# DiltheyLab/MetaMaps

Measured on AMD Instinct MI355X. Metric: Gbp long reads mapped+classified per sec (whole node), miniSeq+H DB, higher is better.
Workload: dtype u32

## Files before the change

### include/metamaps_hip.h

```cpp
#ifndef METAMAPS_HIP_H
#define METAMAPS_HIP_H

#include <stddef.h>
#include <stdint.h>

#ifdef __cplusplus
extern "C" {
#endif

#define MM_ABI_VERSION 6

typedef enum {
  MM_OK = 0,
  MM_ERR_ARG = -1,
  MM_ERR_DEVICE = -2,
  MM_ERR_NOMEM = -3,
  MM_ERR_STATE = -4,
  MM_ERR_LIMIT = -5,
  MM_ERR_NUMERIC = -6,
  MM_ERR_COMM = -7,
  MM_ERR_DATA = -8
} mm_status;

typedef struct mm_ctx mm_ctx;
// ... 130 lines not shown
  int64_t sum_sketch, sum_hits, n_candidates, sum_l2_stream_entries, sum_l2_evals;
  int64_t n_ambiguous_sketch_reads;
  int64_t sum_hits_kept;
  int64_t n_l2_rebuilds;
  int64_t n_l2_wide_redo;
  double ms_minimizer, ms_sketch, ms_probe_gather, ms_sort_hits, ms_l1_scan, ms_l2, ms_compact, ms_total, ms_hit_filter;
  int64_t n_reads_giant;
} mm_map_stats;

int mm_map_batch(mm_ctx* ctx, const mm_index* idx, const mm_seqset* reads, const mm_map_params* p, mm_mapping** out);
int mm_map_batch_phased(mm_ctx* ctx, const mm_index* idx, const mm_seqset* reads, const mm_map_params* p, void (*at_stage)(void* user, int stage), void* user,
                        mm_mapping** out);
int mm_map_batch_reusing(mm_ctx* ctx, const mm_index* idx, const mm_seqset* reads, const mm_map_params* p, const mm_mapping* sketch_of, mm_mapping** out);
int mm_sketch_batch(mm_ctx* ctx, const mm_seqset* reads, const mm_map_params* p, mm_mapping** out);
void mm_mapping_destroy(mm_mapping* m);
int mm_mapping_get_stats(const mm_mapping* m, mm_map_stats* out);
int mm_mapping_release_intermediates(mm_mapping* m);
int mm_mapping_fetch(mm_mapping* m, int64_t* offsets, mm_map_record* records, int64_t cap);
int mm_mapping_add_qualities(mm_ctx* ctx, mm_mapping* m, const mm_seqset* reads, int k);
int mm_mapping_keep_best(mm_ctx* ctx, mm_mapping* m, int k);
int mm_mapping_concat(mm_ctx* ctx, mm_mapping* const* parts, const int32_t* contig_base, int n_parts, mm_mapping** out);
int mm_mapping_from_parts(mm_ctx* ctx, int64_t n_reads, const int32_t* read_len, const mm_map_params* p, int n_parts,
                          const int64_t* const* offsets, const mm_map_record* const* records, const int32_t* contig_base, mm_mapping** out);

int mm_mapping_gather(mm_ctx* ctx, int owner, int64_t n_reads, const int32_t* read_len, const mm_map_params* p, mm_mapping* const* parts, const int32_t* chunk_id,
                      int n_parts, int n_chunks, const int32_t* chunk_rank, const int32_t* contig_base, mm_mapping** out);

int mm_debug_sketch(mm_mapping* m, int64_t* offsets, uint32_t* hash, int32_t* strand, int64_t cap);
int mm_debug_hits(mm_mapping* m, int64_t* offsets, int32_t* contig, int32_t* wpos, int64_t cap);
int mm_debug_candidates(mm_mapping* m, int64_t* offsets, int32_t* triples , int64_t cap);
int mm_debug_l2(mm_mapping* m, int64_t* per_cand , int64_t cap);
int mm_debug_min_hits(mm_mapping* m, int32_t* min_hits );
int mm_debug_probed_lists(mm_mapping* m, const mm_index* idx, int64_t* hist, int32_t n_bins);

int mm_em_create(mm_ctx* ctx, int64_t n_reads, const int64_t* read_off, const int32_t* taxon, const double* mapq,
                 const double* inv_nloc, int32_t n_taxa, mm_em** out);
int mm_em_create_from_mapping(mm_ctx* ctx, const mm_mapping* m, const int32_t* contig_taxon, const int32_t* contig_len, int32_t n_contigs,
                              int32_t n_taxa, mm_em** out);
int mm_em_taxon_counts(mm_em* em, int64_t* counts);
int mm_em_sizes(const mm_em* em, int64_t* n_reads, int64_t* n_entries, int32_t* n_taxa);
void mm_em_destroy(mm_em* em);
int mm_em_iterate(mm_em* em, const double* f, double* f_partial, double* ll_partial);
int mm_em_iterate_allreduce(mm_em* em, const double* f, double* f_next, double* ll);
int mm_em_run(mm_em* em, const double* f0, int max_iter, double* f_out, double* ll_trace, int ll_cap, int* n_iter);
int mm_em_continue(mm_em* em, int max_iter, double* f_out, double* ll_trace, int ll_cap, int* n_iter, int* stopped);
int mm_em_posteriors(mm_em* em, const double* f, double* post , int64_t* best );
int mm_em_bootstrap(mm_em* em, const double* f_start, int32_t rep0, int32_t n_rep, uint64_t seed, const uint8_t* weights,
                    int max_iter, double* f_out, double* ll_out, int32_t* n_iter, int32_t* stopped);
int mm_em_lca(mm_em* em, const double* f, int32_t n_nodes, const int32_t* parent, const int32_t* taxon_node, double threshold,
              int32_t* node_out, double* mass_out, int64_t* direct_out);

int mm_gene_overlap(mm_ctx* ctx, int32_t n_contigs, const int64_t* contig_gene_off, const int32_t* gene_start, const int32_t* gene_stop,
                    const int32_t* gene_group, int32_t n_groups,
                    const int64_t* group_feat_off , const int32_t* group_feat, int32_t n_feats,
                    int64_t n_maps, const int32_t* map_contig, const int32_t* map_start, const int32_t* map_stop, const double* map_ident,
                    int64_t* group_reads , double* group_median ,
                    int64_t* feat_reads , int64_t* maps_on_annotated );

#define MM_COMM_ID_BYTES 128
int mm_comm_unique_id(char id[MM_COMM_ID_BYTES]);
int mm_comm_init(mm_ctx* ctx, const char id[MM_COMM_ID_BYTES], int rank, int nranks);
int mm_comm_info(mm_ctx* ctx, int* n_ranks, int* rank);
int mm_comm_share(mm_ctx* ctx, mm_ctx* owner);
int mm_comm_allreduce_f64(mm_ctx* ctx, double* host_inout, int64_t n);
void mm_comm_destroy(mm_ctx* ctx);

// ... 5 lines not shown
```

### metamaps_amd/capi.py

```python
from __future__ import annotations

import ctypes as C
import os
import re

import numpy as np

_HERE = os.path.dirname(os.path.abspath(__file__))
LIB_PATH = os.path.join(_HERE, "csrc", "libmetamaps_hip.so")
HEADER_PATH = os.path.join(os.path.dirname(_HERE), "include", "metamaps_hip.h")

COMM_ID_BYTES = 128
MM_ERR_ARG = -1
MM_ERR_LIMIT = -5
MM_ERR_DATA = -8


class MMError(RuntimeError):
    def __init__(self, status: int, msg: str):
        super().__init__(f"libmetamaps_hip status {status}: {msg}")
        self.status = status


SEED_STAGE_CB = C.CFUNCTYPE(None, C.c_void_p, C.c_int)
# ... 114 lines not shown
            "mm_index_load": (C.c_int, [vp, C.c_char_p, P(vp)]),
            "mm_index_destroy": (None, [vp]),
            "mm_index_get_info": (C.c_int, [vp, P(IndexInfo)]),
            "mm_index_freq_hist": (C.c_int, [vp, vp, vp, i64, P(i64)]),
            "mm_freq_threshold_from_hist": (C.c_int, [vp, vp, i64, i64, C.c_int]),
            "mm_index_set_freq_threshold": (C.c_int, [vp, C.c_int]),
            "mm_index_entries": (C.c_int, [vp, vp, vp, vp, vp, i64]),
            "mm_index_dup_neighbours": (C.c_int, [vp, vp, vp, i64]),
            "mm_recommended_window": (C.c_int, [f64, C.c_int, f32, C.c_int, u64]),
            "mm_estimate_pvalue": (f64, [C.c_int, C.c_int, f32, C.c_int, u64]),
            "mm_min_hits_relaxed": (C.c_int, [C.c_int, C.c_int, f32]),
            "mm_identity": (None, [C.c_int, C.c_int, C.c_int, P(f32), P(f32)]),
            "mm_map_batch": (C.c_int, [vp, vp, vp, P(MapParams), P(vp)]),
            "mm_map_batch_phased": (C.c_int, [vp, vp, vp, P(MapParams), SEED_STAGE_CB, vp, P(vp)]),
            "mm_map_batch_reusing": (C.c_int, [vp, vp, vp, P(MapParams), vp, P(vp)]),
            "mm_sketch_batch": (C.c_int, [vp, vp, P(MapParams), P(vp)]),
            "mm_mapping_destroy": (None, [vp]),
            "mm_mapping_get_stats": (C.c_int, [vp, P(MapStats)]),
            "mm_comm_info": (C.c_int, [vp, C.POINTER(C.c_int), C.POINTER(C.c_int)]),
            "mm_mapping_gather": (C.c_int, [vp, C.c_int, i64, vp, vp, vp, vp, C.c_int, C.c_int, vp, vp, vp]),
            "mm_mapping_release_intermediates": (C.c_int, [vp]),
            "mm_mapping_fetch": (C.c_int, [vp, vp, vp, i64]),
            "mm_mapping_add_qualities": (C.c_int, [vp, vp, vp, C.c_int]),
            "mm_mapping_concat": (C.c_int, [vp, P(vp), vp, C.c_int, P(vp)]),
            "mm_mapping_keep_best": (C.c_int, [vp, vp, C.c_int]),
            "mm_mapping_from_parts": (C.c_int, [vp, i64, vp, P(MapParams), C.c_int, P(vp), P(vp), vp, P(vp)]),
            "mm_index_plan_chunks": (C.c_int, [vp, vp, u64, vp, i32, P(i32)]),
            "mm_debug_sketch": (C.c_int, [vp, vp, vp, vp, i64]),
            "mm_debug_hits": (C.c_int, [vp, vp, vp, vp, i64]),
            "mm_debug_candidates": (C.c_int, [vp, vp, vp, i64]),
            "mm_debug_l2": (C.c_int, [vp, vp, i64]),
            "mm_debug_min_hits": (C.c_int, [vp, vp]),
            "mm_debug_probed_lists": (C.c_int, [vp, vp, vp, i32]),
            "mm_em_create": (C.c_int, [vp, i64, vp, vp, vp, vp, i32, P(vp)]),
            "mm_em_create_from_mapping": (C.c_int, [vp, vp, vp, vp, i32, i32, P(vp)]),
            "mm_em_taxon_counts": (C.c_int, [vp, vp]),
            "mm_em_sizes": (C.c_int, [vp, P(i64), P(i64), P(i32)]),
            "mm_em_destroy": (None, [vp]),
            "mm_em_iterate": (C.c_int, [vp, vp, vp, P(f64)]),
            "mm_em_iterate_allreduce": (C.c_int, [vp, vp, vp, P(f64)]),
            "mm_em_posteriors": (C.c_int, [vp, vp, vp, vp]),
            "mm_em_run": (C.c_int, [vp, vp, C.c_int, vp, vp, C.c_int, P(C.c_int)]),
            "mm_em_continue": (C.c_int, [vp, C.c_int, vp, vp, C.c_int, P(C.c_int), P(C.c_int)]),
            "mm_em_bootstrap": (C.c_int, [vp, vp, i32, i32, u64, vp, C.c_int, vp, vp, vp, vp]),
            "mm_em_lca": (C.c_int, [vp, vp, i32, vp, vp, f64, vp, vp, vp]),
            "mm_gene_overlap": (C.c_int, [vp, i32, vp, vp, vp, vp, i32, vp, vp, i32, i64, vp, vp, vp, vp, vp, vp, vp, P(i64)]),
            "mm_comm_unique_id": (C.c_int, [C.c_char_p]),
            "mm_comm_init": (C.c_int, [vp, C.c_char_p, C.c_int, C.c_int]),
            "mm_comm_allreduce_f64": (C.c_int, [vp, vp, i64]),
            "mm_comm_share": (C.c_int, [vp, vp]),
            "mm_comm_destroy": (None, [vp]),
        }
        for name, (res, args) in sig.items():
            fn = getattr(L, name)
            fn.restype = res
            fn.argtypes = args
        _lib = L
    return _lib


def _ptr(a):
    return None if a is None else a.ctypes.data_as(C.c_void_p)


class Context:
    def __init__(self, device: int = 0):
# ... 463 lines not shown
        return off, h, s

    def debug_hits(self):
        off = np.zeros(self.n_reads + 1, dtype=np.int64)
        self.ctx.check(lib().mm_debug_hits(self.h, _ptr(off), None, None, 0))
        c = np.zeros(int(off[-1]), dtype=np.int32)
        w = np.zeros(int(off[-1]), dtype=np.int32)
        self.ctx.check(lib().mm_debug_hits(self.h, _ptr(off), _ptr(c), _ptr(w), len(c)))
        return off, c, w

    def debug_candidates(self):
        off = np.zeros(self.n_reads + 1, dtype=np.int64)
        self.ctx.check(lib().mm_debug_candidates(self.h, _ptr(off), None, 0))
        t = np.zeros((int(off[-1]), 3), dtype=np.int32)
        self.ctx.check(lib().mm_debug_candidates(self.h, _ptr(off), _ptr(t), len(t)))
        return off, t

    def debug_l2(self, n_cand: int):
        a = np.zeros((n_cand, 6), dtype=np.int64)
        if n_cand:
            self.ctx.check(lib().mm_debug_l2(self.h, _ptr(a), n_cand))
        return a

    def debug_min_hits(self):
        a = np.zeros(self.n_reads, dtype=np.int32)
        self.ctx.check(lib().mm_debug_min_hits(self.h, _ptr(a)))
        return a

    def debug_probed_lists(self, idx: "Index", n_bins: int = 66) -> np.ndarray:
        a = np.zeros(n_bins, dtype=np.int64)
        self.ctx.check(lib().mm_debug_probed_lists(self.h, idx.h, _ptr(a), n_bins))
        return a

    def close(self):
        if self.h:
            lib().mm_mapping_destroy(self.h)
            self.h = None


class EM:
    def __init__(self, ctx: Context, h, n_taxa: int, n_reads: int, n_entries: int, n_mapped: int | None = None):
        self.ctx, self.h, self.n_taxa, self.n_reads, self.n_entries = ctx, h, n_taxa, n_reads, n_entries
        self.n_mapped = n_mapped

    def iterate(self, f: np.ndarray):
        f = np.ascontiguousarray(f, dtype=np.float64)
        part = np.zeros(self.n_taxa, dtype=np.float64)
        ll = C.c_double()
        self.ctx.check(lib().mm_em_iterate(self.h, _ptr(f), _ptr(part), C.byref(ll)))
        return part, ll.value

    def iterate_allreduce(self, f: np.ndarray):
        f = np.ascontiguousarray(f, dtype=np.float64)
        nxt = np.zeros(self.n_taxa, dtype=np.float64)
        ll = C.c_double()
        self.ctx.check(lib().mm_em_iterate_allreduce(self.h, _ptr(f), _ptr(nxt), C.byref(ll)))
        return nxt, ll.value

    def run(self, f0: np.ndarray, max_iter: int = 1000):
        f0 = np.ascontiguousarray(f0, dtype=np.float64)
        f = np.zeros(self.n_taxa, dtype=np.float64)
        ll = np.zeros(1024, dtype=np.float64)
        n = C.c_int()
        self.ctx.check(lib().mm_em_run(self.h, _ptr(f0), max_iter, _ptr(f), _ptr(ll), len(ll), C.byref(n)))
        return f, ll[:min(n.value, len(ll))]

# ... 53 lines not shown
```

### metamaps_amd/csrc/mm_api.hip

```cpp
#include "mm_env.hpp"
#include "mm_map.hpp"
#include "mm_em.hpp"
#include "mm_stats.hpp"
#include "mm_synth.hpp"
#include "mm_hpc.hpp"
#include "mm_lca.hpp"
#include "mm_gene.hpp"
#include <chrono>
#include <new>
#include <rccl/rccl.h>
#include <rocprim/rocprim.hpp>

namespace mm {
void seqset_upload(mm_seqset* s);
void seqset_upload_nt16(mm_seqset* s);
int64_t bgzf_inflate(mm_ctx* ctx, const uint8_t* comp, int64_t comp_bytes, const int64_t* comp_off, const int32_t* comp_len, int32_t n,
                     uint8_t* out, int64_t out_cap, const int64_t* out_off, int32_t* status);
void bgzf_deflate(mm_ctx* ctx, const uint8_t* in, int64_t in_bytes, uint8_t* out, int64_t out_cap, int64_t* out_bytes, int32_t* n_blocks);
int64_t bgzf_deflate_bound(int64_t in_bytes);
mm_gzip* gzip_open(mm_ctx* ctx, int64_t chunk, int64_t segment);
void gzip_close(mm_gzip* g);
int gzip_feed(mm_gzip* g, const uint8_t* comp, int64_t n, bool last, int64_t* avail);
int64_t gzip_read(mm_gzip* g, uint8_t* out, int64_t cap);
void gzip_stats(const mm_gzip* g, int64_t* counts, double* seconds);
// ... 792 lines not shown
    if (!triples) return;
    MM_REQUIRE(cap >= m->n_cand, MM_ERR_ARG, "output capacity too small");
    m->cand.download(triples, (size_t)(3 * m->n_cand), m->ctx->stream);
    MM_HIP(mm::stream_sync(m->ctx->stream));
  });
}
int mm_debug_l2(mm_mapping* m, int64_t* per_cand, int64_t cap) {
  if (m && m->released) return MM_ERR_STATE;
  if (!m || !per_cand) return MM_ERR_ARG;
  return guarded(m->ctx, [&] {
    MM_REQUIRE(cap >= m->n_cand, MM_ERR_ARG, "output capacity too small");
    auto h = m->l2.to_host(m->ctx->stream, (size_t)m->n_cand);
    for (int64_t i = 0; i < m->n_cand; ++i) {
      per_cand[6 * i] = h[(size_t)i].contig; per_cand[6 * i + 1] = h[(size_t)i].mean_pos; per_cand[6 * i + 2] = h[(size_t)i].shared;
      per_cand[6 * i + 3] = h[(size_t)i].opt_beg; per_cand[6 * i + 4] = h[(size_t)i].opt_end; per_cand[6 * i + 5] = h[(size_t)i].accepted;
    }
  });
}
int mm_debug_min_hits(mm_mapping* m, int32_t* min_hits) {
  if (m && m->released) return MM_ERR_STATE;
  if (!m || !min_hits) return MM_ERR_ARG;
  memcpy(min_hits, m->h_min_hits.data(), m->h_min_hits.size() * sizeof(int32_t));
  return MM_OK;
}

int mm_debug_probed_lists(mm_mapping* m, const mm_index* idx, int64_t* hist, int32_t n_bins) {
  if (m && m->released) return MM_ERR_STATE;
  if (!m || !idx || !hist || n_bins < 3) return MM_ERR_ARG;
  return guarded(m->ctx, [&] {
    MM_HIP(hipSetDevice(m->ctx->device));
    mm::probed_list_hist(m->ctx, idx, m, n_bins, hist);
  });
}

int mm_em_create(mm_ctx* ctx, int64_t n_reads, const int64_t* read_off, const int32_t* taxon, const double* mapq, const double* inv_nloc,
                 int32_t n_taxa, mm_em** out) {
  if (!ctx || !read_off || !out || n_reads < 0 || n_taxa <= 0) return MM_ERR_ARG;
  return guarded(ctx, [&] {
    MM_HIP(hipSetDevice(ctx->device));
    auto* E = new mm_em;
    try { mm::em_create(ctx, n_reads, read_off, taxon, mapq, inv_nloc, n_taxa, E); } catch (...) { delete E; throw; }
    *out = E;
  });
}
int mm_em_create_from_mapping(mm_ctx* ctx, const mm_mapping* m, const int32_t* contig_taxon, const int32_t* contig_len, int32_t n_contigs,
                              int32_t n_taxa, mm_em** out) {
  if (!ctx || !m || !contig_taxon || !contig_len || !out || n_contigs < 0 || n_taxa <= 0) return MM_ERR_ARG;
  return guarded(ctx, [&] {
    MM_HIP(hipSetDevice(ctx->device));
    auto* E = new mm_em;
    try { mm::em_create_from_mapping(ctx, m, contig_taxon, contig_len, n_contigs, n_taxa, E); } catch (...) { delete E; throw; }
    *out = E;
  });
}
int mm_em_taxon_counts(mm_em* em, int64_t* counts) {
  if (!em || !counts) return MM_ERR_ARG;
  return guarded(em->ctx, [&] {
    auto ts = em->tstart.to_host(em->ctx->stream, (size_t)em->n_taxa + 1);
    for (int32_t t = 0; t < em->n_taxa; ++t) counts[t] = ts[(size_t)t + 1] - ts[(size_t)t];
  });
}
int mm_em_sizes(const mm_em* em, int64_t* n_reads, int64_t* n_entries, int32_t* n_taxa) {
  if (!em) return MM_ERR_ARG;
  if (n_reads) *n_reads = em->n_reads;
  if (n_entries) *n_entries = em->n_entries;
  if (n_taxa) *n_taxa = em->n_taxa;
// ... 89 lines not shown
```

### metamaps_amd/csrc/mm_map.hip

```cpp
#include "mm_map.hpp"
#include <functional>
#include <memory>
#include <rocprim/rocprim.hpp>
#include "mm_l2_core.hpp"
#include "mm_size_classes.hpp"
#include "mm_l2.hpp"
#include "mm_l2z.hpp"
#include "mm_l2_dense.hpp"
#include <cstdlib>
#include <atomic>
#include <thread>
#include "mm_stats.hpp"
#include <algorithm>
#include <numeric>
#include "mm_sketch.hpp"
#include "mm_seed.hpp"
#include "mm_l1.hpp"

namespace mm {

namespace {
struct HostLap {
  const bool on = getenv("MM_HOST_TIMING") != nullptr; std::chrono::steady_clock::time_point t = std::chrono::steady_clock::now();
  void operator()(const char* what) { if (!on) return; const auto n = std::chrono::steady_clock::now(); fprintf(stderr, "host %-28s %8.1f us\n", what, std::chrono::duration<double, std::micro>(n - t).count()); t = n; }
// ... 456 lines not shown
  }

  void seed_stage_and_fused() {
    surv.alloc((size_t)n + 1); surv.zero(st);
    std::vector<uint64_t> h_stage_off((size_t)n + 1, 0);
    for (int64_t r = 0; r < n; ++r)
      h_stage_off[(size_t)r + 1] = h_stage_off[(size_t)r] + (M->h_sk_n[(size_t)r] > 0 ? (sw.hf_stage_cap.set ? (uint64_t)sw.hf_stage_cap.v : 1024 + 2 * (uint64_t)M->h_sk_n[(size_t)r]) : 0);
    stage_off.alloc((size_t)n + 1); stage_off.upload(h_stage_off.data(), h_stage_off.size(), st);
    stage.alloc((size_t)std::max<uint64_t>(h_stage_off[(size_t)n], 1));
    MM_HIP(mm::stream_sync(st));
    hl("K3 stage_off loop + upload");
    if (!(sw.use_fused && n_fused > 0)) return;
    const size_t lds = sizeof(SeedFilterStreamLds);
    MM_HIP(hipFuncSetAttribute((const void*)seed_filter_stream_kernel<false>, hipFuncAttributeMaxDynamicSharedMemorySize, (int)lds));
    MM_HIP(hipFuncSetAttribute((const void*)seed_filter_stream_kernel<true>, hipFuncAttributeMaxDynamicSharedMemorySize, (int)lds));
    DBuf<uint32_t> sf_ticket(1);
    sf_ticket.zero(st);
    DBuf<unsigned long long> sf_prof;
    if (sw.sf_prof) { sf_prof.alloc(16); sf_prof.zero(st); }
    int sf_grid = (int)std::min<int64_t>(n, std::max(ctx->cus, 1));
    if (sw.sf_grid.set) sf_grid = std::max(1, std::min(sf_grid, sw.sf_grid.v));
    const size_t t_sf = T.begin(&M->stats.ms_hit_filter);
    if (sf_prof.p)
      seed_filter_stream_kernel<true><<<dim3((unsigned)sf_grid), dim3(SF_THREADS), lds, st>>>(IV, M->sk_hash.p, M->mz.off.p, M->sk_n.p, M->d_read_len.p, M->min_hits.p, surv.p, stage.p, stage_off.p,
                                                                         need_old.p, reinterpret_cast<const uint32_t*>(need_old.p), raw_per_read.p, (int)n, sf_ticket.p, sf_prof.p);
    else
      seed_filter_stream_kernel<false><<<dim3((unsigned)sf_grid), dim3(SF_THREADS), lds, st>>>(IV, M->sk_hash.p, M->mz.off.p, M->sk_n.p, M->d_read_len.p, M->min_hits.p, surv.p, stage.p, stage_off.p,
                                                                         need_old.p, reinterpret_cast<const uint32_t*>(need_old.p), raw_per_read.p, (int)n, sf_ticket.p, nullptr);
    MM_KERNEL_CHECK();
    T.end(t_sf);
    if (sf_prof.p) {
      auto h = sf_prof.to_host(st);
      const double tot = (double)std::accumulate(h.begin(), h.end(), 0ull);
      fprintf(stderr, "MM_SF_PROF share of cycles: zero+top %.3f | next head + resolve %.3f | scan %.3f | lists+count %.3f | window sums+alive+issue %.3f | phase 2 %.3f | survivors+end %.3f | total %.3g cycles over %d workgroups\n",
              h[0] / tot, (h[1] + h[7]) / tot, h[2] / tot, (h[3] + h[8]) / tot, (h[4] + h[9] + h[10] + h[11]) / tot, (h[5] + h[12]) / tot, h[6] / tot, tot, sf_grid);
      fprintf(stderr, "MM_SF_PROF in detail: top %.3f | first answers + second probes issued %.3f, their answers %.3f | scan %.3f | pieces loaded, counted, parked %.3f, next hashes asked for + barrier %.3f | "
                      "window sums %.3f, alive %.3f, barrier %.3f, hashes there + look-ups issued %.3f | bit tests + slots %.3f, barrier %.3f | survivors+end %.3f\n",
              h[0] / tot, h[7] / tot, h[1] / tot, h[2] / tot, h[8] / tot, h[3] / tot, h[9] / tot, h[10] / tot, h[4] / tot, h[11] / tot, h[12] / tot, h[5] / tot, h[6] / tot);
    }
  }

  int64_t hits_of(int64_t r) const { return (int64_t)(M->h_read_hit_off[(size_t)r + 1] - M->h_read_hit_off[(size_t)r]); }

  void sort_hits() {
    if (total_hits > 0) {
      const size_t t_sh = T.begin(&M->stats.ms_sort_hits);
      hl("K4 hits alloc + emit launch");
      int key_bits = 32; while (key_bits < 64 && ((int64_t)1 << (key_bits - 32)) < I->n_contigs) ++key_bits;
      if (sort_hits_radix(key_bits)) sort_hits_segmented(key_bits);
      T.end(t_sh);
    }
    hl("K4 launches + sync");
  }

  bool sort_hits_radix(int key_bits) {
    static_assert(ipt_list_is<1, 2, 3, 4, 6, 8, 12, 16>(HIT_SORT_IPTS), "the dispatch below lists the classes of mm_size_classes.hpp");
    uint64_t left_seen = 0;
    const ReadBins RB = bin_reads(n, N_HIT_SORT_CLASSES, [&](int64_t r) -> int {
      const uint64_t c = (uint64_t)hits_of(r);
      left_seen |= (uint64_t)(c > HIT_SORT_LDS_MAX);
      return hit_sort_class_index(c);
    });
    hl("K4 bin");
    DBuf<int32_t> list(std::max<size_t>(RB.order.size(), 1));
    list.upload(RB.order.data(), RB.order.size(), st);
    hl("K4 list upload");
    size_t at = 0;
    for (auto& run : RB.runs) {
      const int32_t* lp = list.p + at;
      dispatch<1, 2, 3, 4, 6, 8, 12, 16>(HIT_SORT_IPTS[run.first], [&](auto tag) {
        constexpr int IPT = decltype(tag)::value;
// ... 423 lines not shown
    T.collect();
    M->stats.n_mappings = M->n_rec;
    for (int64_t r = 0; r < n; ++r) if (M->h_rec_off[(size_t)r + 1] > M->h_rec_off[(size_t)r]) M->stats.n_reads_mapped++;
  }
};
}

void map_batch(mm_ctx* ctx, const mm_index* I, const mm_seqset* reads, const mm_map_params& P, mm_mapping* M) {
  MapRun R(ctx, I, reads, P, M);
  R.begin();
  R.minimizers();
  R.sketch();
  if (!R.after_sketch()) return;
  R.tiebreak_lists();
  R.thresholds();
  R.seed_hits();
  R.sort_hits();
  R.l1_candidates();
  if (R.ncand > 0) { R.l2(); R.compact(); } else R.no_candidates();
  R.finish();
}

void probed_list_hist(mm_ctx* ctx, const mm_index* I, const mm_mapping* M, int nb, int64_t* hist) {
  hipStream_t st = ctx->stream;
  DBuf<unsigned long long> d((size_t)nb);
  d.zero(st);
  if (M->n_reads > 0)
    probed_list_hist_kernel<<<dim3((unsigned)M->n_reads), dim3(256), 0, st>>>(make_view(I), M->sk_hash.p, M->mz.off.p, M->sk_n.p, nb, d.p);
  MM_KERNEL_CHECK();
  auto h = d.to_host(st);
  for (int i = 0; i < nb; ++i) hist[i] = (int64_t)h[(size_t)i];
}

}
```

### metamaps_amd/csrc/mm_map.hpp

```cpp
#pragma once
#include "mm_common.hpp"
#include "mm_index.hpp"
#include "mm_minimizer.hpp"

namespace mm {
struct L2Result {
  int32_t contig, mean_pos, shared, strand, accepted, pad;
  int64_t opt_beg, opt_end;
  uint32_t n_stream, n_evals, n_rebuilds, pad2;
};
}

struct mm_mapping {
  mm_ctx* ctx = nullptr;
  int64_t n_reads = 0, n_cand = 0, n_rec = 0;
  int smax = 0;
  mm_map_params params{};
  mm_map_stats stats{};
  std::vector<int32_t> read_len;
  std::vector<uint8_t> active;
  void (*at_stage)(void*, int) = nullptr; void* at_stage_user = nullptr;
  const mm_mapping* sketch_donor = nullptr;
  bool sketch_only = false;
  mm::MinimizerSet mz;
  mm::DBuf<uint32_t> sk_hash;
  mm::DBuf<uint8_t> sk_strand;
  mm::DBuf<int32_t> sk_n;
  mm::DBuf<uint8_t> amb;
  std::vector<int32_t> h_sk_n, h_min_hits;
  mm::DBuf<int32_t> min_hits, accept_min, d_read_len;
  mm::DBuf<uint64_t> read_hit_off;
  std::vector<uint64_t> h_read_hit_off;
  mm::DBuf<uint64_t> hits;
  mm::DBuf<uint64_t> cand_off;
  std::vector<uint64_t> h_cand_off;
  mm::DBuf<int32_t> cand;
  mm::DBuf<int32_t> cand_read;
  mm::DBuf<mm::L2Result> l2;
  mm::DBuf<mm_map_record> rec;
  mm::DBuf<uint64_t> rec_off;
  std::vector<uint64_t> h_rec_off;
  bool has_mapq = false;
  bool released = false;
};

namespace mm {
void map_batch(mm_ctx* ctx, const mm_index* I, const mm_seqset* reads, const mm_map_params& P, mm_mapping* M);
void mapping_add_qualities(mm_ctx* ctx, mm_mapping* M, int k);
void probed_list_hist(mm_ctx* ctx, const mm_index* I, const mm_mapping* M, int nb, int64_t* hist);
}
```

### metamaps_amd/csrc/mm_seed.hpp

```cpp
#pragma once
#include "mm_map.hpp"

namespace mm {

__global__ void __launch_bounds__(256) probe_kernel(IndexView I, const uint32_t* __restrict__ sk_hash, const uint64_t* __restrict__ off,
                                                    const int32_t* __restrict__ sk_n, uint32_t* __restrict__ probe_cnt,
                                                    uint64_t* __restrict__ probe_start, const uint8_t* __restrict__ only ) {
  const int r = blockIdx.x;
  if (only && !only[r]) return;
  const uint64_t o = off[r];
  const int s = sk_n[r];
  const int grp = threadIdx.x >> 2, sub = threadIdx.x & 3, gshift = (threadIdx.x & 63) & ~3;
  const ulonglong2* __restrict__ tab = reinterpret_cast<const ulonglong2*>(I.tab);
  const uint64_t tslots = (uint64_t)I.tab_buckets << 2;
  constexpr int NP = 4;
  for (int i0 = grp; i0 < s; i0 += 64 * NP) {
    uint32_t hq[NP]; uint64_t sq[NP]; ulonglong2 vq[NP];
#pragma unroll
    for (int u = 0; u < NP; ++u) { hq[u] = i0 + 64 * u < s ? sk_hash[o + i0 + 64 * u] : 0u; sq[u] = tab_slot(hq[u], I.tab_buckets); }
#pragma unroll
    for (int u = 0; u < NP; ++u) vq[u] = tab[sq[u] + sub];
    auto resolve = [&](uint32_t h, uint64_t slot, ulonglong2 v, bool active, int i) {
      bool pending = active;
      while (__any(pending)) {
// ... 175 lines not shown

constexpr int SF_THREADS = 1024, SF_GROUPS = SF_THREADS / 4;
constexpr int SF_LPG = 11;
constexpr int SF_SMAX = SF_GROUPS * SF_LPG;
constexpr int SF_CHUNKS = 6144;
__device__ __forceinline__ void lds_barrier() { asm volatile("s_waitcnt lgkmcnt(0)\n\ts_barrier" ::: "memory"); }

#ifndef SF_STREAM_WAVES_PER_EU
#define SF_STREAM_WAVES_PER_EU 4
#endif
struct SeedFilterStreamLds {
  uint32_t cnt[HF_SLOTS + HF_PAD_SLOTS];
  uint32_t good[HF_SLOTS / 32], alive[HF_SLOTS / 32 + 4];
  uint32_t lstart8[SF_SMAX];
  uint16_t lcnt[SF_SMAX];
  uint16_t coff8[SF_SMAX + 8];
  uint16_t anchor[SF_CHUNKS / 4];
  uint32_t wsum[SF_THREADS / 64], wsum2[SF_THREADS / 64];
  uint32_t cursor, fallback, total8, hraw, tick[2], pad_[2];
  ulonglong2 codes[SF_CHUNKS];
};
static_assert(sizeof(SeedFilterStreamLds) <= 160 * 1024, "the streaming seed filter's LDS must fit one CU");
template <bool PROF>
__global__ void __launch_bounds__(SF_THREADS) __attribute__((amdgpu_waves_per_eu(SF_STREAM_WAVES_PER_EU, SF_STREAM_WAVES_PER_EU))) seed_filter_stream_kernel(IndexView I, const uint32_t* __restrict__ sk_hash, const uint64_t* __restrict__ off,
                                                                        const int32_t* __restrict__ sk_n, const int32_t* __restrict__ read_len,
                                                                        const int32_t* __restrict__ min_hits, uint32_t* __restrict__ surv_n,
                                                                        uint64_t* __restrict__ stage, const uint64_t* __restrict__ stage_off,
                                                                        uint8_t* need_old, const uint32_t* __restrict__ cls_words ,
                                                                        uint32_t* __restrict__ raw_hits, int n_reads, uint32_t* __restrict__ ticket,
                                                                        unsigned long long* __restrict__ prof ) {
  extern __shared__ __align__(16) unsigned char sf_dyn[];
  SeedFilterStreamLds& L = *reinterpret_cast<SeedFilterStreamLds*>(sf_dyn);
  const ulonglong2* __restrict__ tab = reinterpret_cast<const ulonglong2*>(I.tab);
  const uint64_t tslots = (uint64_t)I.tab_buckets << 2;
  uint32_t hq[SF_LPG]; ulonglong2 vq[SF_LPG];
  int r_cur = 0, s_cur = 0; uint64_t o_cur = 0;
  unsigned long long pt[16] = {0, 0, 0, 0, 0, 0, 0, 0, 0, 0, 0, 0, 0, 0, 0, 0}, pt0 = 0;
  auto lapp = [&](int i) { if (PROF) { const unsigned long long t = __builtin_readcyclecounter(); pt[i] += t - pt0; pt0 = t; } };
  if (PROF) pt0 = __builtin_readcyclecounter();
  
  for (int it = -1; it < 0 || r_cur < n_reads; ++it) {
    int tid = (int)threadIdx.x;
    asm volatile("" : "+v"(tid));
    const int lane = tid & 63, wid = tid >> 6;
    const int grp = tid >> 2, sub = tid & 3, gshift = lane & ~3;
    auto uni64 = [](uint64_t v) { return (uint64_t)(uint32_t)__builtin_amdgcn_readfirstlane((int)(uint32_t)v) | (uint64_t)(uint32_t)__builtin_amdgcn_readfirstlane((int)(uint32_t)(v >> 32)) << 32; };
    auto head = [&](int r, int& s, uint64_t& o) {
      const int rr = min(r, n_reads - 1);
      const uint32_t cw = cls_words[rr >> 2]; const int sn = sk_n[rr]; const uint64_t on = off[rr];
      s = 0; o = 0;
      if (r < n_reads && !((cw >> (8 * (rr & 3))) & 0xffu)) {
        s = sn; o = on;
        if (s <= 0) { s = 0; if (tid == 0) { surv_n[r] = 0; raw_hits[r] = 0; } }
      }
    };
    auto load_hashes = [&](int s_, uint64_t o_) {
      const int su = __builtin_amdgcn_readfirstlane(s_);
      const char* __restrict__ hb = reinterpret_cast<const char*>(sk_hash + uni64(o_));
      const uint32_t last = (uint32_t)max(su - 1, 0);
      if (su > 0) {
#pragma unroll
        for (int u = 0; u < SF_LPG; ++u) hq[u] = *reinterpret_cast<const uint32_t*>(hb + (size_t)(min((uint32_t)(grp + SF_GROUPS * u), last) << 2));
      } else {
#pragma unroll
        for (int u = 0; u < SF_LPG; ++u) hq[u] = 0u;
      }
    };
    auto issue_lookups = [&]() {
#pragma unroll
      for (int u = 0; u < SF_LPG; ++u) asm volatile("" : "+v"(hq[u]));
      int sub_ = (int)threadIdx.x & 3;
      asm volatile("" : "+v"(sub_));
#pragma unroll
      for (int u = 0; u < SF_LPG; ++u) vq[u] = tab[tab_slot(hq[u], I.tab_buckets) + sub_];
    };
    if (it < 0) {
      if (tid == 0) L.tick[0] = atomicAdd(ticket, 1u);
      if (tid < 4) L.alive[HF_SLOTS / 32 + tid] = 0;
      lds_barrier();
      r_cur = __builtin_amdgcn_readfirstlane((int)L.tick[0]);
      head(r_cur, s_cur, o_cur);
      load_hashes(s_cur, o_cur);
      issue_lookups();
      continue;
    }
    if (tid == 0) L.tick[(it + 1) & 1] = atomicAdd(ticket, 1u);
    int r_next = n_reads, s_next = 0; uint64_t o_next = 0;
    bool next_issued = false, next_known = false;
    if (s_cur > 0) {
      const int r = __builtin_amdgcn_readfirstlane(r_cur), s = __builtin_amdgcn_readfirstlane(s_cur);
      const uint64_t stage_base = stage_off[r];
      const uint32_t stage_cap = (uint32_t)(stage_off[r + 1] - stage_base);
      const uint32_t len = (uint32_t)max(read_len[r], 1);
      const int nb = min((int)((len - 1) >> HF_BIN_SHIFT) + 2, HF_SLOTS);
      int m = min_hits[r]; if (m < 1) m = 1;
      {
        uint32_t z = 0;
        asm volatile("" : "+v"(z));
        for (int i = tid; i < (HF_SLOTS + HF_PAD_SLOTS) / 4; i += SF_THREADS) reinterpret_cast<uint4*>(L.cnt)[i] = make_uint4(z, z, z, z);
        if (tid < (int)(sizeof L.lcnt / 16)) reinterpret_cast<uint4*>(L.lcnt)[tid] = make_uint4(z, z, z, z);
        if (tid == 0) { L.cursor = z; L.fallback = z; L.pad_[0] = z; }
      }
      lds_barrier();
      lapp(0);
      r_next = __builtin_amdgcn_readfirstlane((int)L.tick[(it + 1) & 1]);
      head(r_next, s_next, o_next);
      next_known = true;
      auto settle = [&](int i, uint32_t h, const ulonglong2& v, bool pending) -> bool {
        const bool match = pending && v.x != 0 && (uint32_t)v.x == h, empty = pending && v.x == 0;
        const uint32_t done = (uint32_t)(__ballot(match || empty) >> gshift) & 0xfu;
        if (match) {
          const uint32_t cnt = (uint32_t)(v.x >> 32);
          if ((uint64_t)cnt < (uint64_t)(int64_t)I.freq_threshold) {
            if (cnt > 0xffffu) L.fallback = 1;
            L.lcnt[i] = (uint16_t)cnt; L.lstart8[i] = (uint32_t)(v.y >> 3);
          }
        }
        return !pending || done != 0;
      };
      uint32_t pmask = 0;
#pragma unroll
      for (int u = 0; u < SF_LPG; ++u) {
        const int i = grp + SF_GROUPS * u;
        if (!settle(i, hq[u], vq[u], i < s)) { pmask |= 1u << u; vq[u] = tab[tab_next_sector(tab_slot(hq[u], I.tab_buckets), tslots) + sub]; }
      }
      lapp(7);
      if (__any(pmask != 0)) {
#pragma unroll
        for (int u = 0; u < SF_LPG; ++u) {
          const int i = grp + SF_GROUPS * u;
          const uint32_t h = hq[u]; uint64_t slot = tab_next_sector(tab_slot(h, I.tab_buckets), tslots); ulonglong2 v = vq[u];
          bool pending = (pmask >> u) & 1u;
          while (__any(pending)) {
            if (settle(i, h, v, pending)) pending = false;
            if (pending) { slot = tab_next_sector(slot, tslots); v = tab[slot + sub]; }
          }
        }
      }
      lds_barrier();
      lapp(1);
      {
        uint32_t c8[3], hr = 0, mine = 0;
#pragma unroll
        for (int j = 0; j < 3; ++j) { const int i = tid * 3 + j; const uint32_t c = i < s ? L.lcnt[i] : 0u; c8[j] = (c + 7) >> 3; mine += c8[j]; hr += c; }
        const uint32_t inc = (uint32_t)wave_incl_scan((int)mine), inc2 = (uint32_t)wave_incl_scan((int)hr);
        if (lane == 63) { L.wsum[wid] = inc; L.wsum2[wid] = inc2; }
        lds_barrier();
        uint32_t basew = 0, tot = 0, tot2 = 0;
#pragma unroll
        for (int q = 0; q < SF_THREADS / 64; ++q) { const uint32_t x = L.wsum[q]; if (q < wid) basew += x; tot += x; tot2 += L.wsum2[q]; }
        uint32_t ex = basew + inc - mine;
#pragma unroll
        for (int j = 0; j < 3; ++j) {
          const int i = tid * 3 + j;
          if (i <= s) L.coff8[i] = (uint16_t)min(ex, 0xffffu);
          for (uint32_t a = (ex + 3) >> 2, a1 = min((ex + c8[j] + 3) >> 2, (uint32_t)(SF_CHUNKS / 4)); a < a1; ++a) L.anchor[a] = (uint16_t)i;
          ex += c8[j];
        }
        if (tid == 0) { L.total8 = tot; L.hraw = tot2; if (tot > (uint32_t)SF_CHUNKS || tot2 > 65535u) L.fallback = 1; }
      }
      lds_barrier();
      lapp(2);
      if (L.fallback) { if (tid == 0) { need_old[r] = 1; surv_n[r] = 0; raw_hits[r] = 0; } }
      else {
        load_hashes(s_next, o_next);
        {
          constexpr int NP = SF_CHUNKS / SF_THREADS;
          const uint32_t T8u = (uint32_t)__builtin_amdgcn_readfirstlane((int)L.total8);
          ulonglong2 v[NP];
#pragma unroll
          for (int j = 0; j < NP; ++j) {
            v[j] = make_ulonglong2(0, 0);
            if ((uint32_t)(j * SF_THREADS) < T8u) {
              const uint32_t q = min((uint32_t)(tid + j * SF_THREADS), T8u - 1);
              uint32_t li = L.anchor[q >> 2];
              while ((uint32_t)L.coff8[li + 1] <= q) ++li;
              v[j] = *reinterpret_cast<const ulonglong2*>(I.occ16 + ((uint64_t)L.lstart8[li] << 3) + (uint64_t)(q - (uint32_t)L.coff8[li]) * 8u);
            }
          }
#pragma unroll
          for (int j = 0; j < NP; ++j) {
            const uint32_t q = (uint32_t)(tid + j * SF_THREADS);
            if (q < T8u) {
              const ulonglong2 x = v[j];
#pragma unroll
              for (int t = 0; t < 8; ++t) atomicAdd(&L.cnt[(uint32_t)((t < 4 ? x.x : x.y) >> (16 * (t & 3))) & 0xffffu], 1u);
              L.codes[q] = x;
            }
          }
          lapp(8);
        }
        lds_barrier();
        lapp(3);
        {
          const uint32_t* cnt = L.cnt;
#pragma unroll
          for (int kk = 0; kk < HF_SLOTS / SF_THREADS; ++kk) {
            const int b = tid + kk * SF_THREADS;
            uint32_t sum = 0;
            for (int i = 0; i < nb; ++i) sum += cnt[(b + i) & (HF_SLOTS - 1)];
            const uint64_t gb = __ballot(sum >= (uint32_t)m);
            if (lane == 0) { L.good[(b >> 5)] = (uint32_t)gb; L.good[(b >> 5) + 1] = (uint32_t)(gb >> 32); }
          }
        }
        lds_barrier();
        lapp(9);
        if (tid < HF_SLOTS / 32) {
          uint32_t al = 0;
          for (int j = 0; j < nb; ++j) {
            const int wsh = j >> 5, bsh = j & 31;
            const uint32_t g0 = L.good[(tid - wsh) & 255], g1 = L.good[(tid - wsh - 1) & 255];
            al |= bsh ? (g0 << bsh) | (g1 >> (32 - bsh)) : g0;
          }
          L.alive[tid] = al;
        }
        lapp(10);
        lds_barrier();
        lapp(4);
        issue_lookups();
        lapp(11);
        next_issued = true;
        uint64_t* const dst = stage + stage_base;
        uint16_t* const sv = reinterpret_cast<uint16_t*>(L.cnt);
        const uint32_t sv_cap = min(stage_cap, (uint32_t)(2 * (HF_SLOTS + HF_PAD_SLOTS)));
        const uint32_t T8 = L.total8;
        uint32_t cv = 0;
        if (lane == 0) cv = atomicAdd(&L.pad_[0], 1u);
        for (uint32_t c = (uint32_t)__builtin_amdgcn_readfirstlane((int)cv); c * 64u < T8; c = (uint32_t)__builtin_amdgcn_readfirstlane((int)cv)) {
          if (lane == 0) cv = atomicAdd(&L.pad_[0], 1u);
          const uint32_t q = c * 64u + (uint32_t)lane;
          uint32_t mask = 0;
          if (q < T8) {
            const ulonglong2 x = L.codes[q];
#pragma unroll
            for (int t = 0; t < 8; ++t) {
              const uint32_t code = (uint32_t)((t < 4 ? x.x : x.y) >> (16 * (t & 3))) & 0xffffu;
              mask |= ((L.alive[code >> 5] >> (code & 31)) & 1u) << t;
            }
          }
          const int mine = __popc(mask);
          const int incl = wave_incl_scan(mine);
          const int total = __builtin_amdgcn_readlane(incl, 63);
          if (total == 0) continue;
          uint32_t base = 0;
          if (lane == 63) base = atomicAdd(&L.cursor, (uint32_t)total);
          base = (uint32_t)__builtin_amdgcn_readlane((int)base, 63);
          uint32_t pos = base + (uint32_t)(incl - mine);
          while (mask) {
            const int t = __ffs(mask) - 1; mask &= mask - 1;
            if (pos < sv_cap) sv[pos] = (uint16_t)(q << 3 | (uint32_t)t);
            ++pos;
          }
        }
        lapp(12);
        lds_barrier();
        lapp(5);
        const uint32_t n_s = L.cursor;
        if (n_s > sv_cap) { if (tid == 0) { need_old[r] = 1; surv_n[r] = 0; raw_hits[r] = 0; } }
        else {
          for (uint32_t j = tid; j < n_s; j += SF_THREADS) {
            const uint32_t e = sv[j], q = e >> 3;
            uint32_t li = L.anchor[q >> 2];
            while ((uint32_t)L.coff8[li + 1] <= q) ++li;
            dst[j] = I.occ[((uint64_t)L.lstart8[li] << 3) + (uint64_t)(q - (uint32_t)L.coff8[li]) * 8u + (e & 7u)] & ~(uint64_t)(PW_DP | PW_DN);
          }
          if (tid == 0) { surv_n[r] = n_s; raw_hits[r] = L.hraw; }
        }
      }
    }
    if (!next_issued) {
      lds_barrier();
      if (!next_known) { r_next = __builtin_amdgcn_readfirstlane((int)L.tick[(it + 1) & 1]); head(r_next, s_next, o_next); }
      load_hashes(s_next, o_next);
      issue_lookups();
    }
    lds_barrier();
    lapp(6);
    r_cur = r_next; s_cur = s_next; o_cur = o_next;
  }
  if (PROF && threadIdx.x == 0) for (int i = 0; i < 16; ++i) atomicAdd(&prof[i], pt[i]);
}

__global__ void __launch_bounds__(256) move_ranges_kernel(const uint64_t* __restrict__ src, const uint64_t* __restrict__ sb, const uint64_t* __restrict__ se,
                                                          uint64_t* __restrict__ dst, const uint64_t* __restrict__ db) {
  const uint64_t s0 = sb[blockIdx.x], n = se[blockIdx.x] - s0, d0 = db[blockIdx.x];
  for (uint64_t i = threadIdx.x; i < n; i += 256) dst[d0 + i] = src[s0 + i];
}
__global__ void __launch_bounds__(256) sum_u32_kernel(const uint32_t* __restrict__ v, int64_t n, unsigned long long* __restrict__ out) {
  unsigned long long acc = 0;
  for (int64_t i = (int64_t)blockIdx.x * 256 + threadIdx.x; i < n; i += (int64_t)gridDim.x * 256) acc += v[i];
  for (int d = 32; d > 0; d >>= 1) acc += __shfl_xor(acc, d, 64);
  if ((threadIdx.x & 63) == 0 && acc) atomicAdd(out, acc);
}

__global__ void __launch_bounds__(256) probed_list_hist_kernel(IndexView I, const uint32_t* __restrict__ sk_hash, const uint64_t* __restrict__ off,
                                                               const int32_t* __restrict__ sk_n, int nb, unsigned long long* __restrict__ hist) {
  const int r = blockIdx.x, s = sk_n[r];
  const uint64_t o = off[r];
  for (int i = threadIdx.x; i < s; i += 256) {
    uint32_t cnt = 0; uint64_t start = 0;
    int b = 0;
    if (index_find(I, sk_hash[o + i], &cnt, &start)) b = (uint64_t)cnt < (uint64_t)(int64_t)I.freq_threshold ? (int)min(cnt, (uint32_t)(nb - 2)) : nb - 1;
    atomicAdd(&hist[b], 1ull);
  }
}

__global__ void read_hit_bounds_kernel(const uint64_t* __restrict__ off, const uint64_t* __restrict__ hit_off, int64_t n,
                                       uint64_t* __restrict__ read_hit_off) {
  int64_t r = (int64_t)blockIdx.x * blockDim.x + threadIdx.x;
  if (r <= n) read_hit_off[r] = hit_off[off[r]];
}

}
```

Measured before the change: 27.03.

## Issue second-sector hash probes early for next read and serialize deep probes

```diff
diff --git a/include/metamaps_hip.h b/include/metamaps_hip.h
--- a/include/metamaps_hip.h
+++ b/include/metamaps_hip.h
@@ -186,6 +186,7 @@
 int mm_debug_l2(mm_mapping* m, int64_t* per_cand , int64_t cap);
 int mm_debug_min_hits(mm_mapping* m, int32_t* min_hits );
 int mm_debug_probed_lists(mm_mapping* m, const mm_index* idx, int64_t* hist, int32_t n_bins);
+int mm_debug_probe_depth(mm_mapping* m, const mm_index* idx, int32_t* depth, uint8_t* found, int64_t cap);
 
 int mm_em_create(mm_ctx* ctx, int64_t n_reads, const int64_t* read_off, const int32_t* taxon, const double* mapq,
                  const double* inv_nloc, int32_t n_taxa, mm_em** out);
diff --git a/metamaps_amd/capi.py b/metamaps_amd/capi.py
--- a/metamaps_amd/capi.py
+++ b/metamaps_amd/capi.py
@@ -170,6 +170,7 @@
             "mm_debug_l2": (C.c_int, [vp, vp, i64]),
             "mm_debug_min_hits": (C.c_int, [vp, vp]),
             "mm_debug_probed_lists": (C.c_int, [vp, vp, vp, i32]),
+            "mm_debug_probe_depth": (C.c_int, [vp, vp, vp, vp, i64]),
             "mm_em_create": (C.c_int, [vp, i64, vp, vp, vp, vp, i32, P(vp)]),
             "mm_em_create_from_mapping": (C.c_int, [vp, vp, vp, vp, i32, i32, P(vp)]),
             "mm_em_taxon_counts": (C.c_int, [vp, vp]),
@@ -699,6 +700,16 @@
         self.ctx.check(lib().mm_debug_probed_lists(self.h, idx.h, _ptr(a), n_bins))
         return a
 
+    def debug_probe_depth(self, idx: "Index", with_found: bool = False):
+        off = np.zeros(self.n_reads + 1, dtype=np.int64)
+        self.ctx.check(lib().mm_debug_sketch(self.h, _ptr(off), None, None, 0))
+        n = int(off[-1])
+        d = np.zeros(n, dtype=np.int32)
+        f = np.zeros(n, dtype=np.uint8)
+        if n:
+            self.ctx.check(lib().mm_debug_probe_depth(self.h, idx.h, _ptr(d), _ptr(f), n))
+        return (d, f.astype(bool)) if with_found else d
+
     def close(self):
         if self.h:
             lib().mm_mapping_destroy(self.h)
diff --git a/metamaps_amd/csrc/mm_api.hip b/metamaps_amd/csrc/mm_api.hip
--- a/metamaps_amd/csrc/mm_api.hip
+++ b/metamaps_amd/csrc/mm_api.hip
@@ -848,6 +848,17 @@
     mm::probed_list_hist(m->ctx, idx, m, n_bins, hist);
   });
 }
+int mm_debug_probe_depth(mm_mapping* m, const mm_index* idx, int32_t* depth, uint8_t* found, int64_t cap) {
+  if (m && m->released) return MM_ERR_STATE;
+  if (!m || !idx || !depth) return MM_ERR_ARG;
+  return guarded(m->ctx, [&] {
+    MM_HIP(hipSetDevice(m->ctx->device));
+    int64_t tot = 0;
+    for (int64_t r = 0; r < m->n_reads; ++r) tot += m->h_sk_n[(size_t)r];
+    MM_REQUIRE(cap >= tot, MM_ERR_ARG, "output capacity too small");
+    mm::probe_depth(m->ctx, idx, m, depth, found);
+  });
+}
 
 int mm_em_create(mm_ctx* ctx, int64_t n_reads, const int64_t* read_off, const int32_t* taxon, const double* mapq, const double* inv_nloc,
                  int32_t n_taxa, mm_em** out) {
diff --git a/metamaps_amd/csrc/mm_map.hip b/metamaps_amd/csrc/mm_map.hip
--- a/metamaps_amd/csrc/mm_map.hip
+++ b/metamaps_amd/csrc/mm_map.hip
@@ -512,11 +512,11 @@
     if (sf_prof.p) {
       auto h = sf_prof.to_host(st);
       const double tot = (double)std::accumulate(h.begin(), h.end(), 0ull);
-      fprintf(stderr, "MM_SF_PROF share of cycles: zero+top %.3f | next head + resolve %.3f | scan %.3f | lists+count %.3f | window sums+alive+issue %.3f | phase 2 %.3f | survivors+end %.3f | total %.3g cycles over %d workgroups\n",
-              h[0] / tot, (h[1] + h[7]) / tot, h[2] / tot, (h[3] + h[8]) / tot, (h[4] + h[9] + h[10] + h[11]) / tot, (h[5] + h[12]) / tot, h[6] / tot, tot, sf_grid);
-      fprintf(stderr, "MM_SF_PROF in detail: top %.3f | first answers + second probes issued %.3f, their answers %.3f | scan %.3f | pieces loaded, counted, parked %.3f, next hashes asked for + barrier %.3f | "
-                      "window sums %.3f, alive %.3f, barrier %.3f, hashes there + look-ups issued %.3f | bit tests + slots %.3f, barrier %.3f | survivors+end %.3f\n",
-              h[0] / tot, h[7] / tot, h[1] / tot, h[2] / tot, h[8] / tot, h[3] / tot, h[9] / tot, h[10] / tot, h[4] / tot, h[11] / tot, h[12] / tot, h[5] / tot, h[6] / tot);
+      fprintf(stderr, "MM_SF_PROF share of cycles: zero+top %.3f | next head + settle %.3f | scan %.3f | lists+count %.3f | window sums+alive+issue %.3f | phase 2 %.3f | next read's look %.3f | survivors+end %.3f | total %.3g cycles over %d workgroups\n",
+              h[0] / tot, (h[1] + h[7]) / tot, h[2] / tot, (h[3] + h[8]) / tot, (h[4] + h[9] + h[10] + h[11]) / tot, (h[5] + h[12]) / tot, h[13] / tot, h[6] / tot, tot, sf_grid);
+      fprintf(stderr, "MM_SF_PROF in detail: top %.3f | answers settled (one wait, eleven settles) %.3f, third and later sectors + barrier %.3f | scan %.3f | pieces loaded, counted, parked %.3f, next hashes asked for + barrier %.3f | "
+                      "window sums %.3f, alive %.3f, barrier %.3f, hashes there + look-ups issued %.3f | bit tests + slots %.3f, barrier %.3f | next read's answers looked at + second probes issued %.3f | survivors+end %.3f\n",
+              h[0] / tot, h[7] / tot, h[1] / tot, h[2] / tot, h[8] / tot, h[3] / tot, h[9] / tot, h[10] / tot, h[4] / tot, h[11] / tot, h[12] / tot, h[5] / tot, h[13] / tot, h[6] / tot);
     }
   }
 
@@ -1006,4 +1006,22 @@
   for (int i = 0; i < nb; ++i) hist[i] = (int64_t)h[(size_t)i];
 }
 
+void probe_depth(mm_ctx* ctx, const mm_index* I, const mm_mapping* M, int32_t* depth, uint8_t* found) {
+  hipStream_t st = ctx->stream;
+  if (M->n_reads <= 0 || M->sk_hash.n == 0) return;
+  DBuf<int32_t> d(M->sk_hash.n);
+  DBuf<uint8_t> f(M->sk_hash.n);
+  probe_depth_kernel<<<dim3((unsigned)M->n_reads), dim3(256), 0, st>>>(make_view(I), M->sk_hash.p, M->mz.off.p, M->sk_n.p, d.p, f.p);
+  MM_KERNEL_CHECK();
+  const auto hd = d.to_host(st);
+  const auto hf = f.to_host(st);
+  int64_t o = 0;
+  for (int64_t r = 0; r < M->n_reads; ++r)
+    for (int i = 0; i < M->h_sk_n[(size_t)r]; ++i, ++o) {
+      const size_t src = (size_t)M->mz.h_off[(size_t)r] + (size_t)i;
+      depth[o] = hd[src];
+      if (found) found[o] = hf[src];
+    }
 }
+
+}
diff --git a/metamaps_amd/csrc/mm_map.hpp b/metamaps_amd/csrc/mm_map.hpp
--- a/metamaps_amd/csrc/mm_map.hpp
+++ b/metamaps_amd/csrc/mm_map.hpp
@@ -48,4 +48,5 @@
 void map_batch(mm_ctx* ctx, const mm_index* I, const mm_seqset* reads, const mm_map_params& P, mm_mapping* M);
 void mapping_add_qualities(mm_ctx* ctx, mm_mapping* M, int k);
 void probed_list_hist(mm_ctx* ctx, const mm_index* I, const mm_mapping* M, int nb, int64_t* hist);
+void probe_depth(mm_ctx* ctx, const mm_index* I, const mm_mapping* M, int32_t* depth, uint8_t* found);
 }
diff --git a/metamaps_amd/csrc/mm_seed.hpp b/metamaps_amd/csrc/mm_seed.hpp
--- a/metamaps_amd/csrc/mm_seed.hpp
+++ b/metamaps_amd/csrc/mm_seed.hpp
@@ -231,7 +231,6 @@
   extern __shared__ __align__(16) unsigned char sf_dyn[];
   SeedFilterStreamLds& L = *reinterpret_cast<SeedFilterStreamLds*>(sf_dyn);
   const ulonglong2* __restrict__ tab = reinterpret_cast<const ulonglong2*>(I.tab);
-  const uint64_t tslots = (uint64_t)I.tab_buckets << 2;
   uint32_t hq[SF_LPG]; ulonglong2 vq[SF_LPG];
   int r_cur = 0, s_cur = 0; uint64_t o_cur = 0;
   unsigned long long pt[16] = {0, 0, 0, 0, 0, 0, 0, 0, 0, 0, 0, 0, 0, 0, 0, 0}, pt0 = 0;
@@ -253,25 +252,50 @@
         if (s <= 0) { s = 0; if (tid == 0) { surv_n[r] = 0; raw_hits[r] = 0; } }
       }
     };
+    auto rounds_of = [](int s_) { return (__builtin_amdgcn_readfirstlane(s_) + SF_GROUPS - 1) / SF_GROUPS; };
     auto load_hashes = [&](int s_, uint64_t o_) {
       const int su = __builtin_amdgcn_readfirstlane(s_);
-      const char* __restrict__ hb = reinterpret_cast<const char*>(sk_hash + uni64(o_));
+      const char* __restrict__ hb = su > 0 ? reinterpret_cast<const char*>(sk_hash + uni64(o_)) : reinterpret_cast<const char*>(I.tab);
       const uint32_t last = (uint32_t)max(su - 1, 0);
-      if (su > 0) {
-#pragma unroll
-        for (int u = 0; u < SF_LPG; ++u) hq[u] = *reinterpret_cast<const uint32_t*>(hb + (size_t)(min((uint32_t)(grp + SF_GROUPS * u), last) << 2));
-      } else {
-#pragma unroll
-        for (int u = 0; u < SF_LPG; ++u) hq[u] = 0u;
-      }
-    };
-    auto issue_lookups = [&]() {
+#pragma unroll
+      for (int u = 0; u < SF_LPG; ++u) hq[u] = *reinterpret_cast<const uint32_t*>(hb + (size_t)(min((uint32_t)(grp + SF_GROUPS * u), last) << 2));
+    };
+    auto issue_lookups = [&](int s_) {
+      const int nr = rounds_of(s_);
 #pragma unroll
       for (int u = 0; u < SF_LPG; ++u) asm volatile("" : "+v"(hq[u]));
       int sub_ = (int)threadIdx.x & 3;
       asm volatile("" : "+v"(sub_));
 #pragma unroll
-      for (int u = 0; u < SF_LPG; ++u) vq[u] = tab[tab_slot(hq[u], I.tab_buckets) + sub_];
+      for (int u = 0; u < SF_LPG; ++u) {
+        const uint32_t live = u < nr ? 0xffffffffu : 0u;
+        vq[u] = tab[((uint64_t)((uint32_t)(tab_slot(hq[u], I.tab_buckets) >> 2) & live) << 2) + sub_];
+      }
+    };
+    auto sector_of = [&](uint32_t h, uint32_t d) {
+      uint64_t b = (tab_slot(h, I.tab_buckets) >> 2) + d;
+      if (b >= (uint64_t)I.tab_buckets) b -= I.tab_buckets;
+      return b << 2;
+    };
+    auto look = [&](int s_) {
+      const int su = __builtin_amdgcn_readfirstlane(s_);
+      int sub_ = (int)threadIdx.x & 3;
+      asm volatile("" : "+v"(sub_));
+      uint32_t pm = 0;
+#pragma unroll
+      for (int u = 0; u < SF_LPG; ++u) {
+        asm volatile("" : "+v"(vq[u].x));
+        const bool pend = grp + SF_GROUPS * u < su;
+        const bool hit = (vq[u].x == 0) | ((uint32_t)vq[u].x == hq[u]);
+        const uint32_t done = (uint32_t)(__ballot(pend & hit) >> gshift) & 0xfu;
+        pm |= (uint32_t)(pend & (done == 0)) << u;
+      }
+#pragma unroll
+      for (int u = 0; u < SF_LPG; ++u)
+        if ((pm >> u) & 1u) {
+          asm volatile("" : "+v"(hq[u]));
+          vq[u] = tab[sector_of(hq[u], 1u) + sub_];
+        }
     };
     if (it < 0) {
       if (tid == 0) L.tick[0] = atomicAdd(ticket, 1u);
@@ -280,7 +304,8 @@
       r_cur = __builtin_amdgcn_readfirstlane((int)L.tick[0]);
       head(r_cur, s_cur, o_cur);
       load_hashes(s_cur, o_cur);
-      issue_lookups();
+      issue_lookups(s_cur);
+      look(s_cur);
       continue;
     }
     if (tid == 0) L.tick[(it + 1) & 1] = atomicAdd(ticket, 1u);
@@ -317,24 +342,25 @@
         }
         return !pending || done != 0;
       };
-      uint32_t pmask = 0;
-#pragma unroll
-      for (int u = 0; u < SF_LPG; ++u) {
-        const int i = grp + SF_GROUPS * u;
-        if (!settle(i, hq[u], vq[u], i < s)) { pmask |= 1u << u; vq[u] = tab[tab_next_sector(tab_slot(hq[u], I.tab_buckets), tslots) + sub]; }
-      }
+      const int nr = rounds_of(s);
+      uint32_t rem = 0;
+#pragma unroll
+      for (int u = 0; u < SF_LPG; ++u)
+        if (u < nr) {
+          const int i = grp + SF_GROUPS * u;
+          rem |= (uint32_t)!settle(i, hq[u], vq[u], i < s) << u;
+        }
       lapp(7);
-      if (__any(pmask != 0)) {
-#pragma unroll
-        for (int u = 0; u < SF_LPG; ++u) {
-          const int i = grp + SF_GROUPS * u;
-          const uint32_t h = hq[u]; uint64_t slot = tab_next_sector(tab_slot(h, I.tab_buckets), tslots); ulonglong2 v = vq[u];
-          bool pending = (pmask >> u) & 1u;
-          while (__any(pending)) {
-            if (settle(i, h, v, pending)) pending = false;
-            if (pending) { slot = tab_next_sector(slot, tslots); v = tab[slot + sub]; }
-          }
-        }
+      for (uint32_t d = 2; __any(rem != 0);) {
+        const bool open = rem != 0;
+        const int u = open ? __ffs(rem) - 1 : 0;
+        uint32_t h = hq[0];
+#pragma unroll
+        for (int k = 1; k < SF_LPG; ++k) h = u == k ? hq[k] : h;
+        ulonglong2 v = vq[0];
+        if (open) v = tab[sector_of(h, d) + sub];
+        if (settle(grp + SF_GROUPS * u, h, v, open) || d + 1 >= I.tab_buckets) { rem &= rem - 1; d = 2; }
+        else ++d;
       }
       lds_barrier();
       lapp(1);
@@ -366,26 +392,36 @@
         {
           constexpr int NP = SF_CHUNKS / SF_THREADS;
           const uint32_t T8u = (uint32_t)__builtin_amdgcn_readfirstlane((int)L.total8);
-          ulonglong2 v[NP];
-#pragma unroll
-          for (int j = 0; j < NP; ++j) {
-            v[j] = make_ulonglong2(0, 0);
-            if ((uint32_t)(j * SF_THREADS) < T8u) {
+          auto pieces = [&](auto npc) {
+            constexpr int N = decltype(npc)::value;
+            ulonglong2 v[N];
+#pragma unroll
+            for (int j = 0; j < N; ++j) {
               const uint32_t q = min((uint32_t)(tid + j * SF_THREADS), T8u - 1);
               uint32_t li = L.anchor[q >> 2];
               while ((uint32_t)L.coff8[li + 1] <= q) ++li;
               v[j] = *reinterpret_cast<const ulonglong2*>(I.occ16 + ((uint64_t)L.lstart8[li] << 3) + (uint64_t)(q - (uint32_t)L.coff8[li]) * 8u);
             }
-          }
-#pragma unroll
-          for (int j = 0; j < NP; ++j) {
-            const uint32_t q = (uint32_t)(tid + j * SF_THREADS);
-            if (q < T8u) {
-              const ulonglong2 x = v[j];
-#pragma unroll
-              for (int t = 0; t < 8; ++t) atomicAdd(&L.cnt[(uint32_t)((t < 4 ? x.x : x.y) >> (16 * (t & 3))) & 0xffffu], 1u);
-              L.codes[q] = x;
+#pragma unroll
+            for (int j = 0; j < N; ++j) {
+              const uint32_t q = (uint32_t)(tid + j * SF_THREADS);
+              if (q < T8u) {
+                const ulonglong2 x = v[j];
+#pragma unroll
+                for (int t = 0; t < 8; ++t) atomicAdd(&L.cnt[(uint32_t)((t < 4 ? x.x : x.y) >> (16 * (t & 3))) & 0xffffu], 1u);
+                L.codes[q] = x;
+              }
             }
+          };
+          static_assert(NP == 6, "one case per piece round");
+          switch ((T8u + SF_THREADS - 1) / SF_THREADS) {
+            case 1: pieces(std::integral_constant<int, 1>{}); break;
+            case 2: pieces(std::integral_constant<int, 2>{}); break;
+            case 3: pieces(std::integral_constant<int, 3>{}); break;
+            case 4: pieces(std::integral_constant<int, 4>{}); break;
+            case 5: pieces(std::integral_constant<int, 5>{}); break;
+            case 6: pieces(std::integral_constant<int, 6>{}); break;
+            default: break;
           }
           lapp(8);
         }
@@ -416,7 +452,7 @@
         lapp(10);
         lds_barrier();
         lapp(4);
-        issue_lookups();
+        issue_lookups(s_next);
         lapp(11);
         next_issued = true;
         uint64_t* const dst = stage + stage_base;
@@ -454,6 +490,8 @@
         lapp(12);
         lds_barrier();
         lapp(5);
+        look(s_next);
+        lapp(13);
         const uint32_t n_s = L.cursor;
         if (n_s > sv_cap) { if (tid == 0) { need_old[r] = 1; surv_n[r] = 0; raw_hits[r] = 0; } }
         else {
@@ -471,7 +509,8 @@
       lds_barrier();
       if (!next_known) { r_next = __builtin_amdgcn_readfirstlane((int)L.tick[(it + 1) & 1]); head(r_next, s_next, o_next); }
       load_hashes(s_next, o_next);
-      issue_lookups();
+      issue_lookups(s_next);
+      look(s_next);
     }
     lds_barrier();
     lapp(6);
@@ -504,6 +543,24 @@
   }
 }
 
+__global__ void __launch_bounds__(256) probe_depth_kernel(IndexView I, const uint32_t* __restrict__ sk_hash, const uint64_t* __restrict__ off,
+                                                          const int32_t* __restrict__ sk_n, int32_t* __restrict__ depth, uint8_t* __restrict__ found) {
+  const int r = blockIdx.x, s = sk_n[r];
+  const uint64_t o = off[r], tslots = (uint64_t)I.tab_buckets << 2;
+  for (int i = threadIdx.x; i < s; i += 256) {
+    const uint32_t h = sk_hash[o + i];
+    uint64_t slot = tab_slot(h, I.tab_buckets);
+    int d = 0; bool match = false, empty = false;
+    do {
+      ++d;
+      for (int j = 0; j < 4; ++j) { const uint64_t w0 = I.tab[2 * (slot + j)]; match |= w0 != 0 && (uint32_t)w0 == h; empty |= w0 == 0; }
+      slot = tab_next_sector(slot, tslots);
+    } while (!match && !empty);
+    depth[o + i] = d;
+    if (found) found[o + i] = match ? 1 : 0;
+  }
+}
+
 __global__ void read_hit_bounds_kernel(const uint64_t* __restrict__ off, const uint64_t* __restrict__ hit_off, int64_t n,
                                        uint64_t* __restrict__ read_hit_off) {
   int64_t r = (int64_t)blockIdx.x * blockDim.x + threadIdx.x;
```

New measurement: 25.94. -4.0%, worse.
